# mks0601/ExAvatar_RELEASE

Measured on AMD Instinct MI355X. Metric: train iters/sec (fwd+bwd raster) at 1024x1024 / ~150k Gaussians, higher is better.
Workload: dtype f32

## Files before the change

### exavatar_release_amd/csrc/common.h

```cpp
#pragma once
#include <hip/hip_runtime.h>
#include <stdint.h>
#include "../../include/exa_raster.h"
#include "abi_status.h"

namespace exa {

constexpr int TILE = EXA_RASTER_TILE;
constexpr int SUB = 8;
constexpr int CELL_SUBS = 8;
constexpr int CELL = SUB * CELL_SUBS;
constexpr int SUBS_PER_CELL = CELL_SUBS * CELL_SUBS;
constexpr int BLOCK = 256;
constexpr int CHUNK = 1024;
constexpr int MAX_CELLS = 4096;
constexpr int HEADER_BYTES = 2560;

#ifndef EXA_MAX_BATCH
#define EXA_MAX_BATCH 8
#endif
constexpr int MAX_BATCH = EXA_MAX_BATCH;
template <typename T> struct Batch { T v[MAX_BATCH]; };
template <typename T>
inline Batch<T> make_batch(const T* a, int K) {
    Batch<T> b;
    for (int k = 0; k < MAX_BATCH; ++k) b.v[k] = a[k < K ? k : 0];
    return b;
}

#define EXA_TG_1(a) "s"(a)
#define EXA_TG_2(a, ...) "s"(a), EXA_TG_1(__VA_ARGS__)
#define EXA_TG_3(a, ...) "s"(a), EXA_TG_2(__VA_ARGS__)
#define EXA_TG_4(a, ...) "s"(a), EXA_TG_3(__VA_ARGS__)
#define EXA_TG_5(a, ...) "s"(a), EXA_TG_4(__VA_ARGS__)
#define EXA_TG_6(a, ...) "s"(a), EXA_TG_5(__VA_ARGS__)
#define EXA_TG_7(a, ...) "s"(a), EXA_TG_6(__VA_ARGS__)
#define EXA_TG_8(a, ...) "s"(a), EXA_TG_7(__VA_ARGS__)
#define EXA_TG_9(a, ...) "s"(a), EXA_TG_8(__VA_ARGS__)
#define EXA_TG_10(a, ...) "s"(a), EXA_TG_9(__VA_ARGS__)
#define EXA_TG_11(a, ...) "s"(a), EXA_TG_10(__VA_ARGS__)
#define EXA_TG_12(a, ...) "s"(a), EXA_TG_11(__VA_ARGS__)
#define EXA_TG_13(a, ...) "s"(a), EXA_TG_12(__VA_ARGS__)
#define EXA_TG_14(a, ...) "s"(a), EXA_TG_13(__VA_ARGS__)
#define EXA_TG_15(a, ...) "s"(a), EXA_TG_14(__VA_ARGS__)
#define EXA_TG_16(a, ...) "s"(a), EXA_TG_15(__VA_ARGS__)
#define EXA_TG_17(a, ...) "s"(a), EXA_TG_16(__VA_ARGS__)
#define EXA_TG_18(a, ...) "s"(a), EXA_TG_17(__VA_ARGS__)
#define EXA_TG_19(a, ...) "s"(a), EXA_TG_18(__VA_ARGS__)
#define EXA_TG_20(a, ...) "s"(a), EXA_TG_19(__VA_ARGS__)
#define EXA_TG_21(a, ...) "s"(a), EXA_TG_20(__VA_ARGS__)
#define EXA_TG_22(a, ...) "s"(a), EXA_TG_21(__VA_ARGS__)
#define EXA_TG_23(a, ...) "s"(a), EXA_TG_22(__VA_ARGS__)
#define EXA_TG_24(a, ...) "s"(a), EXA_TG_23(__VA_ARGS__)
#define EXA_TG_TOO_MANY(...) "s"(EXA_TOGETHER_takes_at_most_24_values_behind_the_guard)
#define EXA_TG_PICK(_1, _2, _3, _4, _5, _6, _7, _8, _9, _10, _11, _12, _13, _14, _15, _16, _17, _18, _19, _20, _21, _22, _23, _24, \
                    _25, _26, _27, _28, _29, _30, _31, _32, N, ...) N
#define EXA_TOGETHER(guard, ...)                                                                                            \
    asm("" : "+s"(guard)                                                                                                    \
        : EXA_TG_PICK(__VA_ARGS__, EXA_TG_TOO_MANY, EXA_TG_TOO_MANY, EXA_TG_TOO_MANY, EXA_TG_TOO_MANY, EXA_TG_TOO_MANY,      \
                      EXA_TG_TOO_MANY, EXA_TG_TOO_MANY, EXA_TG_TOO_MANY, EXA_TG_24, EXA_TG_23, EXA_TG_22, EXA_TG_21,         \
                      EXA_TG_20, EXA_TG_19, EXA_TG_18, EXA_TG_17, EXA_TG_16, EXA_TG_15, EXA_TG_14, EXA_TG_13, EXA_TG_12,     \
                      EXA_TG_11, EXA_TG_10, EXA_TG_9, EXA_TG_8, EXA_TG_7, EXA_TG_6, EXA_TG_5, EXA_TG_4, EXA_TG_3, EXA_TG_2,  \
                      EXA_TG_1)(__VA_ARGS__))

__device__ __forceinline__ uint32_t uniform_word(uint32_t v) { return (uint32_t)__builtin_amdgcn_readfirstlane((int)v); }
__device__ __forceinline__ float uniform_word(float v) { return __int_as_float(__builtin_amdgcn_readfirstlane(__float_as_int(v))); }
__device__ __forceinline__ uint4 uniform_word(const uint4& v) {
    return make_uint4(uniform_word(v.x), uniform_word(v.y), uniform_word(v.z), uniform_word(v.w));
}

constexpr float NEAR_CULL = 0.2f;
constexpr float LOWPASS = 0.3f;
constexpr float ALPHA_MAX = 0.99f;
constexpr float ALPHA_MIN = 1.0f / 255.0f;
constexpr float T_EPS = 1e-4f;
constexpr float LOG2E = 1.4426950408889634f;

struct alignas(64) Splat {
    float px, py; uint32_t flags; int32_t radius;
    float ca, cb, cc, opacity;
    float r, g, b, depth;
    uint32_t sub_x, sub_y, n_inst, inst_off;
};
static_assert(sizeof(Splat) == 64, "Splat must be one 64-byte line");

#ifndef EXA_PARTIAL_BYTES
#define EXA_PARTIAL_BYTES 40
#endif
constexpr int PARTIAL_BYTES = EXA_PARTIAL_BYTES;
static_assert(PARTIAL_BYTES == 40 || PARTIAL_BYTES == 48 || PARTIAL_BYTES == 64, "partial records: ten floats packed, three rows, or one 64-byte line");
struct PartialWs { float4* rec; };
typedef float partial_v4 __attribute__((ext_vector_type(4), aligned(8)));
typedef float partial_v2 __attribute__((ext_vector_type(2), aligned(8)));
__device__ __forceinline__ char* partial_at(float4* rec, size_t ps) { return reinterpret_cast<char*>(rec) + ps * PARTIAL_BYTES; }
__device__ __forceinline__ const char* partial_at(const float4* rec, size_t ps) { return reinterpret_cast<const char*>(rec) + ps * PARTIAL_BYTES; }
__device__ __forceinline__ void partial_load(const float4* rec, size_t ps, float4& q0, float4& q1, float4& q2) {
    const char* p = partial_at(rec, ps);
    const partial_v4 a = *reinterpret_cast<const partial_v4*>(p), b = *reinterpret_cast<const partial_v4*>(p + 16);
    q0 = make_float4(a.x, a.y, a.z, a.w); q1 = make_float4(b.x, b.y, b.z, b.w);
    if (PARTIAL_BYTES == 40) {
        const partial_v2 c = *reinterpret_cast<const partial_v2*>(p + 32);
        q2 = make_float4(c.x, c.y, 0.f, 0.f);
    } else {
        const partial_v4 c = *reinterpret_cast<const partial_v4*>(p + 32);
        q2 = make_float4(c.x, c.y, c.z, c.w);
    }
}

struct Grid {
    int W, H;
    int gx, gy;
    int sx, sy;
    int cx, cy, cells;
    int subtiles;
};
__host__ __device__ inline Grid make_grid(int W, int H) {
    Grid g;
    g.W = W; g.H = H;
    g.gx = (W + TILE - 1) / TILE;
    g.gy = (H + TILE - 1) / TILE;
    g.sx = (W + SUB - 1) / SUB;
    g.sy = (H + SUB - 1) / SUB;
    g.cx = (W + CELL - 1) / CELL;
    g.cy = (H + CELL - 1) / CELL;
    g.cells = g.cx * g.cy;
    g.subtiles = g.cells * SUBS_PER_CELL;
    return g;
}

__host__ __device__ inline int num_chunks(int P) { return (P + CHUNK - 1) / CHUNK; }

#ifndef EXA_BIN_PARTS
#define EXA_BIN_PARTS 4
#endif
constexpr int BIN_PARTS = EXA_BIN_PARTS;
struct TileWs {
    ExaRasterHeader* header;
    uint32_t* cls_cur;
    uint32_t* bwd_meta;
    unsigned long long* chunk_cell;
    unsigned long long* cell_cnt;
    uint2* cell_off;
    uint32_t* chunk_inst;
    uint32_t* chunk_vis;
    uint32_t* chunk_tiles;
    uint32_t* chunk_off;
    uint4* cell_desc;
    uint2* ranges;
    uint4* slots;
    uint2* fwd_exit;
    uint32_t* cell_long;
    uint32_t* part_cnt;
    uint4* part_desc;
    uint8_t* cls_code;
};
__host__ __device__ inline uint64_t tile_ws_bytes(int cells, int chunks) {
    return HEADER_BYTES + align256(uint64_t(chunks) * cells * 8) + align256(uint64_t(cells) * 8) +
           align256(uint64_t(cells + 1) * 8) + 4 * align256(uint64_t(chunks + 1) * 4) +
           align256(uint64_t(cells) * 16) + align256(uint64_t(cells) * SUBS_PER_CELL * 8) +
           align256(uint64_t(cells) * SUBS_PER_CELL * 16) + align256(uint64_t(cells) * SUBS_PER_CELL * 8) +
           align256(uint64_t(cells) * BIN_PARTS * SUBS_PER_CELL * 4) + align256(uint64_t(cells) * 4) +
           align256(uint64_t(cells) * BIN_PARTS * 16) + align256(uint64_t(cells) * SUBS_PER_CELL);
}
__host__ __device__ inline TileWs carve_tile_ws(void* base, int cells, int chunks) {
    char* p = static_cast<char*>(base);
    TileWs w;
    w.header = reinterpret_cast<ExaRasterHeader*>(p);
    w.cls_cur = reinterpret_cast<uint32_t*>(p + 256);
    w.bwd_meta = reinterpret_cast<uint32_t*>(p + 128);
    p += HEADER_BYTES;
    w.chunk_cell = reinterpret_cast<unsigned long long*>(p); p += align256(uint64_t(chunks) * cells * 8);
    w.cell_cnt = reinterpret_cast<unsigned long long*>(p); p += align256(uint64_t(cells) * 8);
    w.cell_off = reinterpret_cast<uint2*>(p); p += align256(uint64_t(cells + 1) * 8);
    w.chunk_inst = reinterpret_cast<uint32_t*>(p); p += align256(uint64_t(chunks + 1) * 4);
    w.chunk_vis = reinterpret_cast<uint32_t*>(p); p += align256(uint64_t(chunks + 1) * 4);
    w.chunk_tiles = reinterpret_cast<uint32_t*>(p); p += align256(uint64_t(chunks + 1) * 4);
    w.chunk_off = reinterpret_cast<uint32_t*>(p); p += align256(uint64_t(chunks + 1) * 4);
    w.cell_desc = reinterpret_cast<uint4*>(p); p += align256(uint64_t(cells) * 16);
    w.ranges = reinterpret_cast<uint2*>(p); p += align256(uint64_t(cells) * SUBS_PER_CELL * 8);
    w.slots = reinterpret_cast<uint4*>(p); p += align256(uint64_t(cells) * SUBS_PER_CELL * 16);
    w.fwd_exit = reinterpret_cast<uint2*>(p); p += align256(uint64_t(cells) * SUBS_PER_CELL * 8);
    w.part_cnt = reinterpret_cast<uint32_t*>(p); p += align256(uint64_t(cells) * BIN_PARTS * SUBS_PER_CELL * 4);
    w.cell_long = reinterpret_cast<uint32_t*>(p); p += align256(uint64_t(cells) * 4);
    w.part_desc = reinterpret_cast<uint4*>(p); p += align256(uint64_t(cells) * BIN_PARTS * 16);
    w.cls_code = reinterpret_cast<uint8_t*>(p);
    return w;
}

constexpr int BATCH = 64;
__host__ __device__ inline uint64_t bin_zero_bytes(uint64_t cap) {
    return align256((cap / BATCH + 1) * 16) + align256((cap / BATCH + 1) * 8) + align256(cap);
}
__host__ __device__ inline uint64_t bin_ws_bytes(uint64_t cap) {
    return align256(cap * 8) + align256(cap * 4) + align256(cap * 16) + bin_zero_bytes(cap) +
           align256((cap / BATCH + 1) * 5 * 64 * 4);
}
struct BinWs {
    unsigned long long* keys; uint32_t* sorted; uint4* bucket;
    uint4* owner; unsigned long long* bmask; uint8_t* touched;
    float* ckpt;
};
__host__ __device__ inline BinWs carve_bin_ws(void* base, uint64_t cap) {
    BinWs b;
    char* p = static_cast<char*>(base);
    b.keys = reinterpret_cast<unsigned long long*>(p); p += align256(cap * 8);
    b.sorted = reinterpret_cast<uint32_t*>(p); p += align256(cap * 4);
    b.bucket = reinterpret_cast<uint4*>(p); p += align256(cap * 16);
    b.owner = reinterpret_cast<uint4*>(p); p += align256((cap / BATCH + 1) * 16);
    b.bmask = reinterpret_cast<unsigned long long*>(p); p += align256((cap / BATCH + 1) * 8);
    b.touched = reinterpret_cast<uint8_t*>(p); p += align256(cap);
    b.ckpt = reinterpret_cast<float*>(p);
    return b;
}
__host__ __device__ inline uint32_t cell_slots(uint32_t inst) {
    return inst ? (inst + BATCH - 1) / BATCH + 2 * SUBS_PER_CELL : 0u;
}

__host__ __device__ inline uint64_t grad_ws_bytes(uint64_t cap) { return align256(cap * PARTIAL_BYTES); }
constexpr int GROUP_SCRATCH_FLOATS = 23;
__host__ __device__ inline uint64_t group_scratch_bytes(uint64_t P) { return align256(P * GROUP_SCRATCH_FLOATS * sizeof(float)); }
__host__ __device__ inline PartialWs carve_grad_ws(void* base, uint64_t) {
    PartialWs w;
    w.rec = reinterpret_cast<float4*>(base);
    return w;
}

constexpr int ORDER_CLASSES = 64;
#ifndef EXA_XCD_REGIONS
#define EXA_XCD_REGIONS 8
#endif
constexpr int XCD_REGIONS = EXA_XCD_REGIONS;
static_assert(XCD_REGIONS == 8 || XCD_REGIONS == 1, "eight XCDs, or no regions at all");
__device__ __forceinline__ int xcd_region(int local) { return XCD_REGIONS == 8 ? ((local >> 1) & 3) | ((local >> 3) & 4) : 0; }
constexpr uint32_t BWD_ORDER_MAGIC = 0xB07DE7EDu;
constexpr int BWD_ORDER_DEPTH = 16;
__device__ __forceinline__ int length_class(uint32_t n) { return n ? min(ORDER_CLASSES - 1, (int)((n + 15) / 16)) : 0; }

struct SubTile { int st, cell, local, ox, oy, gsx, gsy; };
__device__ __forceinline__ SubTile decode_subtile(int st, const Grid& g) {
    SubTile s;
    s.st = st;
    s.cell = st >> 6;
    s.local = st & 63;
    const int cxi = s.cell % g.cx, cyi = s.cell / g.cx;
    s.gsx = cxi * CELL_SUBS + (s.local & 7);
    s.gsy = cyi * CELL_SUBS + (s.local >> 3);
    s.ox = s.gsx * SUB;
    s.oy = s.gsy * SUB;
    return s;
}

__device__ __forceinline__ float gauss_power2(float A, float B, float C, float dx, float dy) {
#pragma clang fp contract(off)
    return __builtin_fmaf(A * dx, dx, __builtin_fmaf(C * dy, dy, (B * dx) * dy));
}
__device__ __forceinline__ float gauss_falloff2(float power2) { return __builtin_amdgcn_exp2f(power2); }

struct Footprint { float kA, ysr, X2, D4; bool test; };
__device__ __forceinline__ float clampf(float v, float lo, float hi) { return __builtin_amdgcn_fmed3f(v, lo, hi); }
__device__ __forceinline__ Footprint make_footprint(float A, float B, float C, float opacity, float xm, float ym) {
    Footprint f;
    const float rA = __builtin_amdgcn_rcpf(A), rC = __builtin_amdgcn_rcpf(C);
    const float As = A - 0.25f * B * B * rC;
    f.test = A < 0.f && C < 0.f && As < 0.f;
    const float mag = fabsf(A) * xm * xm + fabsf(B) * xm * ym + fabsf(C) * ym * ym;
    const float thr = -__log2f(255.0f * opacity) - 1e-3f - 1e-5f * mag;
    f.kA = -0.5f * B * rA;
    f.ysr = -0.5f * B * rC * __builtin_amdgcn_sqrtf(thr * __builtin_amdgcn_rcpf(As));
    f.X2 = thr * rA;
    f.D4 = C * As * rA * rA;
    return f;
}
__device__ __forceinline__ bool footprint_band(const Footprint& f, float yl, float yh, float& xa, float& xb) {
    const float yR = clampf(f.ysr, yl, yh), yL = clampf(-f.ysr, yl, yh);
    const float hR2 = f.X2 - f.D4 * yR * yR, hL2 = f.X2 - f.D4 * yL * yL;
    if (hR2 < 0.f || hL2 < 0.f) return false;
    xb = f.kA * yR + __builtin_amdgcn_sqrtf(hR2);
    xa = f.kA * yL - __builtin_amdgcn_sqrtf(hL2);
    return true;
}
__device__ __forceinline__ void wave_lds_fence() {
    asm volatile("s_waitcnt lgkmcnt(0)" ::: "memory");
    __builtin_amdgcn_wave_barrier();
}
struct PreprocessArgs {
    int P, sh_M, sh_degree;
    Grid grid;
    float tanfovx, tanfovy, focal_x, focal_y, scale_modifier;
// ... 135 lines not shown
```

### exavatar_release_amd/csrc/render_fwd.hip

```cpp
#include <stdlib.h>
#include "blend.h"

namespace exa {

constexpr int RBLOCK = 64;

constexpr int SORT_TILE = 2048;
constexpr int SBLOCK = 256;

template <int E>
__device__ __forceinline__ void lds_merge_sort(const unsigned long long* gkeys, int n, uint32_t* __restrict__ sorted,
                                               unsigned long long* keys_out, unsigned long long* buf, int tid) {
    constexpr int NPAD = SBLOCK * E;
    const int lane = tid & 63;
    unsigned long long key[E];
#pragma unroll
    for (int e = 0; e < E; ++e) {
        const int i = e * SBLOCK + tid;
        key[e] = i < n ? gkeys[i] : ~0ull;
        buf[i] = key[e];
    }
    __syncthreads();
    {
        uint32_t rank[E];
// ... 11 lines not shown
        }
        __syncthreads();
#pragma unroll
        for (int e = 0; e < E; ++e) {
            const int i = e * SBLOCK + tid;
            const uint32_t r = (i >= n) ? (uint32_t)lane : rank[e];
            buf[(i & ~63) + r] = key[e];
        }
    }
    __syncthreads();
#pragma unroll
    for (int L = 64, steps = 7; L < NPAD; L <<= 1, ++steps) {
        uint32_t lohi[E];
#pragma unroll
        for (int e = 0; e < E; ++e) {
            key[e] = buf[e * SBLOCK + tid];
            lohi[e] = (uint32_t)L << 16;
        }
        for (int it = 0; it < steps; ++it) {
#pragma unroll
            for (int e = 0; e < E; ++e) {
                const int i = e * SBLOCK + tid;
                const int base = i & ~(2 * L - 1);
                const bool first = (i - base) < L;
                const int p0 = base + (first ? L : 0);
                const int lo = lohi[e] & 0xffff, hi = lohi[e] >> 16;
                const int mid = (lo + hi) >> 1;
                const bool act = lo < hi;
                const unsigned long long pk = buf[p0 + min(mid, L - 1)];
                const bool less = first ? (pk < key[e]) : (pk <= key[e]);
                const int nlo = (act && less) ? mid + 1 : lo;
                const int nhi = (act && !less) ? mid : hi;
                lohi[e] = (uint32_t)nlo | ((uint32_t)nhi << 16);
            }
        }
        __syncthreads();
#pragma unroll
        for (int e = 0; e < E; ++e) {
            const int i = e * SBLOCK + tid;
            const int base = i & ~(2 * L - 1);
            const int off = i - base;
            buf[base + (off < L ? off : off - L) + (int)(lohi[e] & 0xffff)] = key[e];
        }
        __syncthreads();
    }
#pragma unroll
    for (int e = 0; e < E; ++e) {
        const int i = e * SBLOCK + tid;
        if (i < n) {
            sorted[i] = (uint32_t)buf[i];
            if (keys_out) keys_out[i] = buf[i];
        }
    }
}

constexpr int BUCKET_MAX = 48;
template <int E>
__device__ __forceinline__ bool lds_bucket_sort(const unsigned long long* gkeys, int n, uint32_t* __restrict__ sorted,
                                                unsigned long long* keys_out, unsigned long long* buf, uint32_t* cnt,
                                                uint32_t* s_misc, int tid) {
    constexpr int NB = SBLOCK * E;
    const int lane = tid & 63, wave = tid >> 6;
    unsigned long long key[E];
    uint32_t dmin = 0xffffffffu, dmax = 0u;
#pragma unroll
    for (int e = 0; e < E; ++e) key[e] = gkeys[min(e * SBLOCK + tid, n - 1)];
#pragma unroll
    for (int e = 0; e < E; ++e) {
        const int i = e * SBLOCK + tid;
        if (i < n) {
            const uint32_t d = (uint32_t)(key[e] >> 32);
            dmin = min(dmin, d); dmax = max(dmax, d);
        } else {
            key[e] = ~0ull;
        }
        cnt[i] = 0u;
    }
#pragma unroll
    for (int d = 32; d > 0; d >>= 1) {
        dmin = min(dmin, (uint32_t)__shfl_xor((int)dmin, d, 64));
        dmax = max(dmax, (uint32_t)__shfl_xor((int)dmax, d, 64));
    }
    if (lane == 0) { s_misc[wave] = dmin; s_misc[4 + wave] = dmax; }
    __syncthreads();
    dmin = min(min(s_misc[0], s_misc[1]), min(s_misc[2], s_misc[3]));
    dmax = max(max(s_misc[4], s_misc[5]), max(s_misc[6], s_misc[7]));
    const float fmin = __uint_as_float(dmin);
    const float scale = (float)(NB - 1) / fmaxf(__uint_as_float(dmax) - fmin, 1e-30f);
    uint32_t bkt[E], slot[E];
#pragma unroll
    for (int e = 0; e < E; ++e) {
        bkt[e] = 0u; slot[e] = 0u;
        if (e * SBLOCK + tid < n) {
            const float f = (__uint_as_float((uint32_t)(key[e] >> 32)) - fmin) * scale;
            bkt[e] = (uint32_t)min(NB - 1, (int)f);
            slot[e] = __hip_atomic_fetch_add(&cnt[bkt[e]], 1u, __ATOMIC_RELAXED, __HIP_MEMORY_SCOPE_WORKGROUP);
        }
    }
    __syncthreads();
    uint32_t c[E], sum = 0u, mx = 0u;
#pragma unroll
    for (int e = 0; e < E; ++e) { c[e] = cnt[tid * E + e]; sum += c[e]; mx = max(mx, c[e]); }
    uint32_t incl = sum;
#pragma unroll
    for (int d = 1; d < 64; d <<= 1) {
        const uint32_t o = (uint32_t)__shfl_up((int)incl, d, 64);
        if (lane >= d) incl += o;
    }
#pragma unroll
    for (int d = 32; d > 0; d >>= 1) mx = max(mx, (uint32_t)__shfl_xor((int)mx, d, 64));
    if (lane == 63) s_misc[8 + wave] = incl;
    if (lane == 0) s_misc[12 + wave] = mx;
    __syncthreads();
    mx = max(max(s_misc[12], s_misc[13]), max(s_misc[14], s_misc[15]));
    if (mx > (uint32_t)BUCKET_MAX) return false;
    uint32_t run = incl - sum;
    for (int w2 = 0; w2 < wave; ++w2) run += s_misc[8 + w2];
#pragma unroll
    for (int e = 0; e < E; ++e) { cnt[tid * E + e] = run; run += c[e]; }
    __syncthreads();
#pragma unroll
    for (int e = 0; e < E; ++e)
        if (e * SBLOCK + tid < n) buf[cnt[bkt[e]] + slot[e]] = key[e];
    __syncthreads();
#pragma unroll
    for (int e = 0; e < E; ++e) {
        if (e * SBLOCK + tid < n) {
            const uint32_t s0 = cnt[bkt[e]], s1 = bkt[e] + 1u < (uint32_t)NB ? cnt[bkt[e] + 1u] : (uint32_t)n;
            uint32_t rank = s0;
            for (uint32_t j = s0; j < s1; ++j) rank += buf[j] < key[e] ? 1u : 0u;
            sorted[rank] = (uint32_t)key[e];
            if (keys_out) keys_out[rank] = key[e];
        }
    }
    return true;
}

__device__ __forceinline__ void wave_rank_sort64(const unsigned long long* gkeys, int n, uint32_t* __restrict__ sorted,
                                                 unsigned long long* keys_out, unsigned long long* buf, int lane) {
    const unsigned long long mine = lane < n ? gkeys[lane] : ~0ull;
    buf[lane] = mine;
    wave_lds_fence();
    const ulonglong2* s2 = reinterpret_cast<const ulonglong2*>(buf);
    uint32_t rank = 0;
#pragma unroll 8
    for (int j = 0; j < 32; ++j) {
        const ulonglong2 kk = s2[j];
        rank += (kk.x < mine) ? 1u : 0u;
        rank += (kk.y < mine) ? 1u : 0u;
    }
    if (lane < n) {
        sorted[rank] = (uint32_t)mine;
        if (keys_out) keys_out[rank] = mine;
    }
}

template <int R>
__device__ __forceinline__ void rank_sort_list(const unsigned long long* __restrict__ gkeys, int n, int first,
                                               uint32_t* __restrict__ sorted, unsigned long long* s_keys, int tid) {
    unsigned long long mine[R];
    uint32_t rank[R];
#pragma unroll
    for (int r = 0; r < R; ++r) {
        const int i = first + r * SBLOCK + tid;
        mine[r] = i < n ? gkeys[i] : ~0ull;
        rank[r] = 0;
    }
    for (int tile = 0; tile < n; tile += SORT_TILE) {
        const int tn = min(SORT_TILE, n - tile);
        __syncthreads();
        for (int i = tid; i < ((tn + 1) & ~1); i += SBLOCK) s_keys[i] = i < tn ? gkeys[tile + i] : ~0ull;
        __syncthreads();
        const ulonglong2* s2 = reinterpret_cast<const ulonglong2*>(s_keys);
#pragma unroll 4
        for (int j = 0; j < (tn + 1) / 2; ++j) {
            const ulonglong2 kk = s2[j];
#pragma unroll
            for (int r = 0; r < R; ++r) {
                rank[r] += (kk.x < mine[r]) ? 1u : 0u;
                rank[r] += (kk.y < mine[r]) ? 1u : 0u;
            }
        }
    }
#pragma unroll
    for (int r = 0; r < R; ++r)
        if (first + r * SBLOCK + tid < n) sorted[rank[r]] = (uint32_t)mine[r];
}

constexpr int ORDER_WGS = 32;
constexpr int ORDER_BINS = XCD_REGIONS * ORDER_CLASSES;
constexpr int ORDER_LDS_WORDS = 3 * ORDER_BINS + XCD_REGIONS * (BWD_ORDER_DEPTH + 1);
template <typename RangeOf>
__device__ __forceinline__ void order_slots(const TileWs& w, uint32_t* __restrict__ bwd_order, int subtiles, int part, int tid,
                                            uint32_t* __restrict__ lds, RangeOf range_of) {
    uint32_t* const s_off = lds;
    uint32_t* const s_cnt = lds + ORDER_BINS;
    uint32_t* const s_base = lds + 2 * ORDER_BINS;
    uint32_t* const s_bbase = lds + 3 * ORDER_BINS;
    const int lane = tid & 63;
#ifdef EXA_PROBE_SORTLINE
#define ORDER_STAMP(ph) do { if (tid == 0) w.part_cnt[2 * (subtiles + ORDER_WGS) + part * 8 + (ph)] = (uint32_t)wall_clock64(); } while (0)
#else
#define ORDER_STAMP(ph) do {} while (0)
#endif
    ORDER_STAMP(0);
    for (int i = tid; i < ORDER_BINS; i += SBLOCK) s_cnt[i] = 0u;
    __syncthreads();
    const uint4* __restrict__ codes = reinterpret_cast<const uint4*>(w.cls_code);
    const int n16 = subtiles / 16;
    for (int base = 0; base < n16; base += SBLOCK * 4) {
        uint4 v[4];
#pragma unroll
        for (int i = 0; i < 4; ++i) {
            const int idx = base + i * SBLOCK + tid;
            v[i] = idx < n16 ? codes[idx] : make_uint4(0u, 0u, 0u, 0u);
        }
#pragma unroll
        for (int i = 0; i < 4; ++i) {
            const int idx = base + i * SBLOCK + tid;
            const uint32_t word[4] = {v[i].x, v[i].y, v[i].z, v[i].w};
            if ((word[0] | word[1] | word[2] | word[3]) == 0u) continue;
#pragma unroll
            for (int j = 0; j < 16; ++j) {
                const uint32_t cls = (word[j >> 2] >> (8 * (j & 3))) & 0xffu;
                if (cls) atomicAdd(&s_cnt[xcd_region((idx & 3) * 16 + j) * ORDER_CLASSES + cls], 1u);
            }
        }
    }
    __syncthreads();
    ORDER_STAMP(1);
    {
        constexpr int RPW = (XCD_REGIONS + SBLOCK / 64 - 1) / (SBLOCK / 64);
        const int cls = lane == 63 ? 0 : 63 - lane;
        uint32_t v[RPW], incl[RPW];
#pragma unroll
        for (int j = 0; j < RPW; ++j) {
            const int x = (tid >> 6) + j * (SBLOCK / 64);
            v[j] = incl[j] = x < XCD_REGIONS ? s_cnt[x * ORDER_CLASSES + cls] : 0u;
        }
#pragma unroll
        for (int d = 1; d < 64; d <<= 1) {
#pragma unroll
            for (int j = 0; j < RPW; ++j) {
                const uint32_t o = __shfl_up(incl[j], d, 64);
                if (lane >= d) incl[j] += o;
            }
        }
#pragma unroll
        for (int j = 0; j < RPW; ++j) {
            const int x = (tid >> 6) + j * (SBLOCK / 64);
            if (x < XCD_REGIONS) s_off[x * ORDER_CLASSES + cls] = incl[j] - v[j];
        }
    }
    __syncthreads();
    for (int i = tid; i < ORDER_BINS; i += SBLOCK) s_cnt[i] = 0u;
    if (tid < XCD_REGIONS) {
        uint32_t more[BWD_ORDER_DEPTH];
#pragma unroll
        for (int b = 0; b < BWD_ORDER_DEPTH; ++b) more[b] = s_off[tid * ORDER_CLASSES + 4 * b];
        uint32_t run = 0u;
#pragma unroll
        for (int b = 0; b < BWD_ORDER_DEPTH; ++b) { s_bbase[tid * (BWD_ORDER_DEPTH + 1) + b] = run; run += more[b]; }
        s_bbase[tid * (BWD_ORDER_DEPTH + 1) + BWD_ORDER_DEPTH] = run;
    }
    __syncthreads();
    uint32_t M[XCD_REGIONS];
#pragma unroll
    for (int x = 0; x < XCD_REGIONS; ++x) M[x] = s_bbase[x * (BWD_ORDER_DEPTH + 1) + BWD_ORDER_DEPTH];
    uint32_t m_min = M[0], deep_base = M[0];
#pragma unroll
    for (int x = 1; x < XCD_REGIONS; ++x) { m_min = min(m_min, M[x]); deep_base += M[x]; }
    if (part == 0 && tid == 0) { w.bwd_meta[0] = deep_base; w.bwd_meta[2] = bwd_order ? BWD_ORDER_MAGIC : 0u; }
    ORDER_STAMP(2);
    const int per = (subtiles + ORDER_WGS - 1) / ORDER_WGS;
    const int lo = part * per, hi = min(subtiles, lo + per);
    for (int base = lo; base < hi; base += SBLOCK * 4) {
        uint2 r[4];
        uint32_t rank[4];
#pragma unroll
        for (int i = 0; i < 4; ++i) {
            const int st = base + i * SBLOCK + tid;
            r[i] = st < hi ? range_of(st) : make_uint2(0u, 0u);
        }
#pragma unroll
        for (int i = 0; i < 4; ++i) {
            const int st = base + i * SBLOCK + tid;
            const bool valid = st < hi;
            const int cls = length_class(r[i].y - r[i].x), x = xcd_region(st & 63);
            const bool is_empty = valid && cls == 0;
            unsigned long long mine = 0ull;
#pragma unroll
            for (int xr = 0; xr < XCD_REGIONS; ++xr) {
                const unsigned long long m = __ballot(is_empty && x == xr);
                if (x == xr) mine = m;
            }
            const int leader = is_empty ? __ffsll((long long)mine) - 1 : lane;
            uint32_t b0 = 0u;
            if (cls) b0 = atomicAdd(&s_cnt[x * ORDER_CLASSES + cls], 1u);
            else if (is_empty && lane == leader) b0 = atomicAdd(&s_cnt[x * ORDER_CLASSES], (uint32_t)__popcll(mine));
            b0 = (uint32_t)__shfl((int)b0, leader, 64);
            rank[i] = b0 + (is_empty ? (uint32_t)__popcll(mine & ((1ull << lane) - 1ull)) : 0u);
        }
        ORDER_STAMP(3);
        __syncthreads();
        {
            constexpr int BPT = (ORDER_BINS + SBLOCK - 1) / SBLOCK;
            uint32_t c[BPT], got[BPT];
#pragma unroll
            for (int j = 0; j < BPT; ++j) c[j] = j * SBLOCK + tid < ORDER_BINS ? s_cnt[j * SBLOCK + tid] : 0u;
#pragma unroll
            for (int j = 0; j < BPT; ++j) got[j] = c[j] ? atomicAdd(&w.cls_cur[j * SBLOCK + tid], c[j]) : 0u;
#pragma unroll
            for (int j = 0; j < BPT; ++j)
                if (j * SBLOCK + tid < ORDER_BINS) s_base[j * SBLOCK + tid] = s_off[j * SBLOCK + tid] + got[j];
        }
        __syncthreads();
        ORDER_STAMP(4);
#pragma unroll
        for (int i = 0; i < 4; ++i) {
            const int st = base + i * SBLOCK + tid;
            if (st < hi) {
                const int cls = length_class(r[i].y - r[i].x), x = xcd_region(st & 63);
                const uint32_t k = s_base[x * ORDER_CLASSES + cls] + rank[i];
                w.slots[k * XCD_REGIONS + x] = make_uint4(r[i].x, r[i].y, (uint32_t)st, 0u);
                const uint32_t nb = (r[i].y - r[i].x + BATCH - 1) / BATCH, slot0 = r[i].x / BATCH;
                for (uint32_t b = 0; bwd_order && b < nb; ++b) {
                    uint32_t q;
                    if (b < (uint32_t)BWD_ORDER_DEPTH) {
                        const uint32_t kb = s_bbase[x * (BWD_ORDER_DEPTH + 1) + b] + k;
                        q = kb * XCD_REGIONS + (uint32_t)x;
                        if (kb >= m_min) {
                            q = 0u;
#pragma unroll
                            for (int xo = 0; xo < XCD_REGIONS; ++xo) q += min(M[xo], kb) + (xo < x && M[xo] > kb ? 1u : 0u);
                        }
                    } else {
                        q = deep_base + atomicAdd(&w.bwd_meta[1], 1u);
                    }
                    bwd_order[q] = slot0 + b;
                }
            }
        }
        __syncthreads();
        for (int i = tid; i < ORDER_BINS; i += SBLOCK) s_cnt[i] = 0u;
        __syncthreads();
        ORDER_STAMP(5);
    }
#undef ORDER_STAMP
}

__global__ __launch_bounds__(SBLOCK) void sort_short_kernel(Batch<RenderFwdArgs> batch) {
    __shared__ __attribute__((aligned(16))) unsigned long long s_buf[(SBLOCK / 64) * 64];
    const RenderFwdArgs& a = batch.v[blockIdx.y];
    const int wave = threadIdx.x >> 6, lane = threadIdx.x & 63;
    const int idx = (int)blockIdx.x * (SBLOCK / 64) + wave;
    if (idx >= a.grid.subtiles) return;
    if (idx >= (int)a.tw.header->active_cells * SUBS_PER_CELL) return;
    const int st = (int)a.tw.cell_desc[idx >> 6].x * SUBS_PER_CELL + (idx & 63);
    const uint2 range = a.tw.ranges[st];
    const int n = (int)(range.y - range.x);
    if (n > 0 && n <= 64)
        wave_rank_sort64(a.bw.keys + range.x, n, a.bw.sorted + range.x, a.keep_sorted_keys ? a.bw.keys + range.x : nullptr,
                         s_buf + wave * 64, lane);
}

template <bool SPLIT, bool KEEP>
__global__ __launch_bounds__(SBLOCK) __attribute__((amdgpu_waves_per_eu(6, 6))) void sort_subtiles_kernel(Batch<RenderFwdArgs> batch) {
    __shared__ __attribute__((aligned(16))) unsigned long long s_buf[SORT_TILE];
    __shared__ uint32_t s_cnt[SORT_TILE];
    __shared__ uint32_t s_misc[16];
    const RenderFwdArgs& a = batch.v[blockIdx.y];
    if ((int)blockIdx.x >= a.grid.subtiles + ORDER_WGS) return;
    const int tid = threadIdx.x;
#ifdef EXA_PROBE_SORTLINE
    struct TL { const RenderFwdArgs& a; unsigned long long t0; int tid;
        __device__ ~TL() { __syncthreads(); if (tid == 0) { a.tw.part_cnt[2 * blockIdx.x] = (uint32_t)t0; a.tw.part_cnt[2 * blockIdx.x + 1] = (uint32_t)wall_clock64(); } } } tl{a, (unsigned long long)wall_clock64(), tid};
#endif
    if (blockIdx.x < ORDER_WGS) {
        static_assert(ORDER_LDS_WORDS <= SORT_TILE, "order_slots borrows the bucket counters of the sort");
        order_slots(a.tw, a.store_ctx ? reinterpret_cast<uint32_t*>(a.bw.bucket) : nullptr, a.grid.subtiles, (int)blockIdx.x, tid,
                    s_cnt, [&](int st) { return a.tw.ranges[st]; });
        return;
    }
#ifdef EXA_PROBE_SORT
    const unsigned long long t0 = __builtin_readcyclecounter();
#endif
    if (blockIdx.x == ORDER_WGS && tid == 0 && (uint64_t)a.tw.header->num_rendered > a.capacity) a.tw.header->overflow = 1u;
    const int wg = (int)blockIdx.x - ORDER_WGS;
    if (wg >= (int)a.tw.header->active_cells * SUBS_PER_CELL) return;
    if (SPLIT && a.tw.cell_long[wg >> 6] == 0u) return;
    const int st = (int)a.tw.cell_desc[wg >> 6].x * SUBS_PER_CELL + (wg & 63);
    const uint2 range = a.tw.ranges[st];
    const int n = (int)(range.y - range.x);
    if (n == 0) return;
    unsigned long long* gkeys = a.bw.keys + range.x;
    uint32_t* sorted = a.bw.sorted + range.x;
    unsigned long long* const keys_out = KEEP ? gkeys : nullptr;
    if (n <= 64) {
        if (!SPLIT && tid < 64) wave_rank_sort64(gkeys, n, sorted, keys_out, s_buf, tid);
        return;
    }
    if (n > SORT_TILE) {
        for (int first = 0; first < n; first += 8 * SBLOCK) rank_sort_list<8>(gkeys, n, first, sorted, s_buf, tid);
        if (keys_out) {
            __threadfence_block();
            __syncthreads();
            for (int i = tid; i < n; i += SBLOCK) {
                const uint32_t id = sorted[i];
                keys_out[i] = ((unsigned long long)__float_as_uint(a.splats[id].depth) << 32) | id;
            }
        }
        return;
    }
    bool done;
    if (n <= 256) done = lds_bucket_sort<1>(gkeys, n, sorted, keys_out, s_buf, s_cnt, s_misc, tid);
    else if (n <= 512) done = lds_bucket_sort<2>(gkeys, n, sorted, keys_out, s_buf, s_cnt, s_misc, tid);
    else if (n <= 1024) done = lds_bucket_sort<4>(gkeys, n, sorted, keys_out, s_buf, s_cnt, s_misc, tid);
    else done = lds_bucket_sort<8>(gkeys, n, sorted, keys_out, s_buf, s_cnt, s_misc, tid);
    if (done) return;
    __syncthreads();
    if (n <= 256) lds_merge_sort<1>(gkeys, n, sorted, keys_out, s_buf, tid);
    else if (n <= 512) lds_merge_sort<2>(gkeys, n, sorted, keys_out, s_buf, tid);
    else if (n <= 1024) lds_merge_sort<4>(gkeys, n, sorted, keys_out, s_buf, tid);
    else lds_merge_sort<8>(gkeys, n, sorted, keys_out, s_buf, tid);
#ifdef EXA_PROBE_SORT
    __syncthreads();
    if (tid == 0) a.tw.part_cnt[st] = (uint32_t)(__builtin_readcyclecounter() - t0);
#endif
}

template <bool STORE, bool TWO>
__global__ __launch_bounds__(RBLOCK) void render_fwd_kernel(Batch<RenderFwdArgs> batch) {
    __shared__ BatchLds s_b;

    const RenderFwdArgs& a = batch.v[blockIdx.y];
    int subtiles = a.grid.subtiles;
    const int gW = a.grid.W, gH = a.grid.H, gcx = a.grid.cx;
    const uint4* __restrict__ slots = a.tw.slots;
    const Splat* __restrict__ splats = a.splats;
    const uint32_t* __restrict__ sorted_all = a.bw.sorted;
    float* ckpt_all = a.bw.ckpt;
    unsigned long long* bmask = a.bw.bmask;
    uint2* fwd_exit = a.tw.fwd_exit;
    const float* __restrict__ bg = a.bg;
    float* out_color = a.out_color; float* out_depth = a.out_depth; float* out_alpha = a.out_alpha;
    const uint2* ranges = a.tw.ranges;
    const Splat* __restrict__ splats2 = a.splats2;
    const float* src_color = a.src_color; const float* src_depth = a.src_depth; const float* src_alpha = a.src_alpha;
    const float* src_bg = a.src_bg;
    if (TWO)
        EXA_TOGETHER(subtiles, gW, gH, gcx, slots, splats, sorted_all, ckpt_all, bmask, fwd_exit, bg, out_color, out_depth, out_alpha,
                     ranges, splats2, src_color, src_depth, src_alpha, src_bg);
    else
        EXA_TOGETHER(subtiles, gW, gH, gcx, slots, splats, sorted_all, ckpt_all, bmask, fwd_exit, bg, out_color, out_depth, out_alpha);
    if ((int)blockIdx.x >= subtiles) return;
    const int lane = threadIdx.x;
#ifdef EXA_PROBE_FWD
    const unsigned long long t0 = wall_clock64();
#endif
    uint4 slot = uniform_word(slots[blockIdx.x]);
    const float bg0 = uniform_word(bg[0]), bg1 = uniform_word(bg[1]), bg2 = uniform_word(bg[2]);
    EXA_TOGETHER(slot.z, slot.x, slot.y, slot.w, bg0, bg1, bg2);
    Grid grid;
    grid.W = gW; grid.H = gH; grid.cx = gcx;
    const SubTile sub = decode_subtile((int)slot.z, grid);
    const int st = sub.st;
    if (sub.ox >= gW || sub.oy >= gH) return;
    const int pxi = sub.ox + (lane & 7), pyi = sub.oy + (lane >> 3);
    const bool inside = pxi < gW && pyi < gH;
    const float fx = (float)pxi, fy = (float)pyi;
    const uint2 range = TWO ? ranges[slot.z] : make_uint2(slot.x, slot.y);
    const int n = (int)(range.y - range.x);
    if (TWO && n == 0 && reuse_a_pixels(src_color, src_bg, bg0, bg1, bg2)) {
        if (inside) {
            const size_t HW = (size_t)gW * gH, pix = (size_t)pyi * gW + pxi;
            const float c0 = src_color[pix], c1 = src_color[HW + pix], c2 = src_color[2 * HW + pix];
            const float d = src_depth[pix], al = src_alpha[pix];
            out_color[pix] = c0; out_color[HW + pix] = c1; out_color[2 * HW + pix] = c2;
            out_depth[pix] = d; out_alpha[pix] = al;
        }
        if (STORE && lane == 0) fwd_exit[st] = make_uint2(0u, 0u);
        return;
    }

    float T = inside ? 1.0f : 0.0f, Tdead = 1.0f;
    v2f Crg = {0.f, 0.f}, Cbd = {0.f, 0.f};
    const uint32_t* __restrict__ sorted = sorted_all + range.x;
    auto record = [&](uint32_t id) -> const float4* {
        if (TWO) return reinterpret_cast<const float4*>(((id & SRC_B) ? splats2 : splats) + (id & ~SRC_B));
        return reinterpret_cast<const float4*>(splats + id);
    };

    uint32_t id_next = 0;
    float2 r0 = make_float2(0.f, 0.f);
    float4 r1 = make_float4(0.f, 0.f, 0.f, 0.f), r2 = r1;
    if (n > 0) {
        const uint32_t id0 = lane < n ? sorted[lane] : 0u;
        if (64 + lane < n) id_next = sorted[64 + lane];
        if (lane < n) {
            const float4* rec = record(id0);
            r0 = *reinterpret_cast<const float2*>(rec); r1 = rec[1]; r2 = rec[2];
        }
    }
    float* ckpt = ckpt_all + (size_t)(range.x / BATCH) * (5 * 64) + lane;
    int entered = 0;
    for (int base = 0; base < n; base += 64) {
        if (__all(T == 0.0f)) break;
        if (STORE && base > 0) {
            float* c = ckpt + (size_t)entered * (5 * 64);
            c[0] = T > 0.0f ? T : -Tdead; c[64] = Crg.x; c[128] = Crg.y; c[192] = Cbd.x; c[256] = Cbd.y;
        }
        ++entered;
        const unsigned long long unsafe = __builtin_amdgcn_ballot_w64(!conic_safe(r1.x, r1.y, r1.z));
        stage_splat(s_b, lane, r0, r1, r2);
        {
            const int jn = base + 64 + lane;
            r0 = make_float2(0.f, 0.f); r1 = make_float4(0.f, 0.f, 0.f, 0.f); r2 = r1;
            if (jn < n) {
                const float4* rec = record(id_next);
                r0 = *reinterpret_cast<const float2*>(rec); r1 = rec[1]; r2 = rec[2];
            }
            if (jn + 64 < n) id_next = sorted[jn + 64];
        }
        wave_lds_fence();
        const int cnt = min(64, n - base);
        unsigned long long blended = 0ull;
        auto blend4 = [&](const Alpha4& e, const float4& c0, const float4& c1, const float4& c2, const float4& c3, int k) -> bool {
#ifdef EXA_FWD_SKIP_VOTE
            const float amax = fmaxf(fmaxf(e.alpha[0], e.alpha[1]), fmaxf(e.alpha[2], e.alpha[3])) * T;
            if (!__any(amax > 0.0f)) return false;
#endif
            const unsigned long long live_mask = __builtin_amdgcn_ballot_w64(T > 0.0f);
            if (STORE) {
                auto vote_bit = [&](int j, uint32_t bit) -> uint32_t {
                    const unsigned long long m = e.took[j] & live_mask;
                    uint32_t r;
                    asm("s_cmp_lg_u64 %1, 0\n\ts_cselect_b32 %0, %2, 0" : "=s"(r) : "s"(m), "s"(bit) : "scc");
                    return r;
                };
                const uint32_t nib = vote_bit(0, 1u) | vote_bit(1, 2u) | vote_bit(2, 4u) | vote_bit(3, 8u);
                blended |= (unsigned long long)nib << k;
            }
            float Tb[4], w[4];
            blend_group4(T, Tdead, live_mask, e.alpha, Tb, w);
            Crg = __builtin_elementwise_fma(v2f{c0.x, c0.y}, v2f{w[0], w[0]}, Crg);
            Cbd = __builtin_elementwise_fma(v2f{c0.z, c0.w}, v2f{w[0], w[0]}, Cbd);
            Crg = __builtin_elementwise_fma(v2f{c1.x, c1.y}, v2f{w[1], w[1]}, Crg);
            Cbd = __builtin_elementwise_fma(v2f{c1.z, c1.w}, v2f{w[1], w[1]}, Cbd);
            Crg = __builtin_elementwise_fma(v2f{c2.x, c2.y}, v2f{w[2], w[2]}, Crg);
            Cbd = __builtin_elementwise_fma(v2f{c2.z, c2.w}, v2f{w[2], w[2]}, Cbd);
            Crg = __builtin_elementwise_fma(v2f{c3.x, c3.y}, v2f{w[3], w[3]}, Crg);
            Cbd = __builtin_elementwise_fma(v2f{c3.z, c3.w}, v2f{w[3], w[3]}, Cbd);
#ifdef EXA_FWD_EXIT4
            return __all(T == 0.0f);
#else
            return (k & 4) ? __all(T == 0.0f) : false;
#endif
        };
        auto group4 = [&](const Ops4& ops, int k) -> bool {
            const float4 c0 = s_b.col[k], c1 = s_b.col[k + 1], c2 = s_b.col[k + 2], c3 = s_b.col[k + 3];
            Alpha4 e = splat_alpha4(ops, fx, fy, true);
            if ((unsafe >> k) & 0xfull) power_guard4(e, ops, (uint32_t)((unsafe >> k) & 0xfull));
            return blend4(e, c0, c1, c2, c3, k);
        };
        Ops4 opsA = load_ops4(s_b, 0);
        for (int k = 0; k < cnt; k += 8) {
            const Ops4 opsB = load_ops4(s_b, (k + 4) & 63);
            if (group4(opsA, k)) break;
            if (k + 4 >= cnt) break;
            opsA = load_ops4(s_b, (k + 8) & 63);
            if (group4(opsB, k + 4)) break;
        }
        if (STORE && lane == 0) bmask[range.x / BATCH + (uint32_t)(entered - 1)] = blended;
        wave_lds_fence();
    }

    const size_t HW = (size_t)gW * gH;
    if (inside) {
        const size_t pix = (size_t)pyi * gW + pxi;
        const float Tf = T > 0.0f ? T : Tdead;
        out_color[pix] = Crg.x + Tf * bg0;
        out_color[HW + pix] = Crg.y + Tf * bg1;
        out_color[2 * HW + pix] = Cbd.x + Tf * bg2;
        out_depth[pix] = Cbd.y;
        out_alpha[pix] = 1.0f - Tf;
    }
    if (STORE) {
        if (lane == 0) fwd_exit[st] = make_uint2((uint32_t)n, (uint32_t)entered);
#ifdef EXA_PROBE_FWD
        if (lane == 0) {
            a.tw.part_cnt[4 * blockIdx.x] = (uint32_t)t0;
            a.tw.part_cnt[4 * blockIdx.x + 1] = (uint32_t)wall_clock64();
            const uint32_t hw = __builtin_amdgcn_s_getreg((31 << 11) | 4), xcc = __builtin_amdgcn_s_getreg((31 << 11) | 20);
            a.tw.part_cnt[4 * blockIdx.x + 2] = (hw & 0xffffu) | ((xcc & 0xfu) << 16);
        }
#endif
        if (n > 0) {
            float* c = ckpt + (size_t)((n + BATCH - 1) / BATCH) * (5 * 64);
            c[0] = T > 0.0f ? T : Tdead; c[64] = Crg.x; c[128] = Crg.y; c[192] = Cbd.x; c[256] = Cbd.y;
        }
    }
}

static int max_subtiles(const RenderFwdArgs* a, int K) {
    int n = 0;
    for (int k = 0; k < K; ++k) n = max(n, a[k].grid.subtiles);
    return n;
}

hipError_t launch_sort_subtiles(const RenderFwdArgs* a, int K, hipStream_t s) {
    const int subtiles = max_subtiles(a, K);
    if (subtiles == 0) return hipSuccess;
    const int split_at = dev_knobs().split_subtiles;
    bool keep = false;
    for (int k = 0; k < K; ++k) keep = keep || a[k].keep_sorted_keys != 0;
    const dim3 grid(subtiles + ORDER_WGS, K);
    if (subtiles >= split_at) {
        sort_short_kernel<<<dim3((subtiles + SBLOCK / 64 - 1) / (SBLOCK / 64), K), SBLOCK, 0, s>>>(make_batch(a, K));
        if (keep) sort_subtiles_kernel<true, true><<<grid, SBLOCK, 0, s>>>(make_batch(a, K));
        else sort_subtiles_kernel<true, false><<<grid, SBLOCK, 0, s>>>(make_batch(a, K));
    } else {
        if (keep) sort_subtiles_kernel<false, true><<<grid, SBLOCK, 0, s>>>(make_batch(a, K));
        else sort_subtiles_kernel<false, false><<<grid, SBLOCK, 0, s>>>(make_batch(a, K));
    }
    return hipGetLastError();
}

#ifndef EXA_FWD_LDS_PAD
#define EXA_FWD_LDS_PAD 0
#endif
hipError_t launch_render_fwd(const RenderFwdArgs* a, int K, hipStream_t s) {
    const int subtiles = max_subtiles(a, K);
    if (subtiles == 0) return hipSuccess;
    constexpr int pad = EXA_FWD_LDS_PAD;
    if (a[0].splats2) {
        if (a[0].store_ctx) render_fwd_kernel<true, true><<<dim3(subtiles, K), RBLOCK, (size_t)pad, s>>>(make_batch(a, K));
        else render_fwd_kernel<false, true><<<dim3(subtiles, K), RBLOCK, (size_t)pad, s>>>(make_batch(a, K));
    } else if (a[0].store_ctx)
        render_fwd_kernel<true, false><<<dim3(subtiles, K), RBLOCK, (size_t)pad, s>>>(make_batch(a, K));
    else
        render_fwd_kernel<false, false><<<dim3(subtiles, K), RBLOCK, (size_t)pad, s>>>(make_batch(a, K));
    return hipGetLastError();
}

}
```

Measured before the change: 7950.

## Sort small subtile lists per wave and long lists via owner-indexed tail workgroups

Adds a quads sort kernel that is used on the non-split path by default. It packs four subtiles per workgroup, one per wave, and sorts lists of up to 512 keys inside a single wave with a new wave-level bucket sort that falls back to a rank sort. Longer lists are handed to extra tail workgroups that find their lists through the owner slot table. The goal is to stop spending a whole 256-thread workgroup with barriers on each small subtile list. In exchange the grid is sized from capacity, so many tail blocks may exit early, and per-wave LDS regions add pressure.

```diff
diff --git a/exavatar_release_amd/csrc/common.h b/exavatar_release_amd/csrc/common.h
--- a/exavatar_release_amd/csrc/common.h
+++ b/exavatar_release_amd/csrc/common.h
@@ -134,6 +134,11 @@
 #define EXA_BIN_PARTS 4
 #endif
 constexpr int BIN_PARTS = EXA_BIN_PARTS;
+#ifndef EXA_WAVE_KEYS
+#define EXA_WAVE_KEYS 512
+#endif
+constexpr int WAVE_KEYS = EXA_WAVE_KEYS;
+static_assert(WAVE_KEYS == 0 || WAVE_KEYS == 256 || WAVE_KEYS == 512, "EXA_WAVE_KEYS: 0, 256 or 512");
 struct TileWs {
     ExaRasterHeader* header;
     uint32_t* cls_cur;
diff --git a/exavatar_release_amd/csrc/render_fwd.hip b/exavatar_release_amd/csrc/render_fwd.hip
--- a/exavatar_release_amd/csrc/render_fwd.hip
+++ b/exavatar_release_amd/csrc/render_fwd.hip
@@ -187,6 +187,108 @@
     if (lane < n) {
         sorted[rank] = (uint32_t)mine;
         if (keys_out) keys_out[rank] = mine;
+    }
+}
+
+template <int E>
+__device__ __forceinline__ void wave_rank_sort_staged(const unsigned long long (&key)[E], int n, uint32_t* __restrict__ sorted,
+                                                      unsigned long long* keys_out, unsigned long long* buf, int lane) {
+#pragma unroll
+    for (int e = 0; e < E; ++e) buf[e * 64 + lane] = key[e];
+    wave_lds_fence();
+    uint32_t rank[E];
+#pragma unroll
+    for (int e = 0; e < E; ++e) rank[e] = 0u;
+    const ulonglong2* s2 = reinterpret_cast<const ulonglong2*>(buf);
+#pragma unroll 2
+    for (int j = 0; j < (n + 1) / 2; ++j) {
+        const ulonglong2 kk = s2[j];
+#pragma unroll
+        for (int e = 0; e < E; ++e) {
+            rank[e] += (kk.x < key[e]) ? 1u : 0u;
+            rank[e] += (kk.y < key[e]) ? 1u : 0u;
+        }
+    }
+#pragma unroll
+    for (int e = 0; e < E; ++e) {
+        if (e * 64 + lane < n) {
+            sorted[rank[e]] = (uint32_t)key[e];
+            if (keys_out) keys_out[rank[e]] = key[e];
+        }
+    }
+}
+
+template <int E>
+__device__ __forceinline__ void wave_bucket_sort(const unsigned long long* gkeys, int n, uint32_t* __restrict__ sorted,
+                                                 unsigned long long* keys_out, unsigned long long* buf, uint32_t* cnt, int lane) {
+    constexpr int NB = 64 * E;
+    unsigned long long key[E];
+    uint32_t dmin = 0xffffffffu, dmax = 0u;
+#pragma unroll
+    for (int e = 0; e < E; ++e) key[e] = gkeys[min(e * 64 + lane, n - 1)];
+#pragma unroll
+    for (int e = 0; e < E; ++e) {
+        const int i = e * 64 + lane;
+        if (i < n) {
+            const uint32_t d = (uint32_t)(key[e] >> 32);
+            dmin = min(dmin, d); dmax = max(dmax, d);
+        } else {
+            key[e] = ~0ull;
+        }
+        cnt[i] = 0u;
+    }
+#pragma unroll
+    for (int d = 32; d > 0; d >>= 1) {
+        dmin = min(dmin, (uint32_t)__shfl_xor((int)dmin, d, 64));
+        dmax = max(dmax, (uint32_t)__shfl_xor((int)dmax, d, 64));
+    }
+    wave_lds_fence();
+    const float fmin = __uint_as_float(dmin);
+    const float scale = (float)(NB - 1) / fmaxf(__uint_as_float(dmax) - fmin, 1e-30f);
+    uint32_t bs[E];
+#pragma unroll
+    for (int e = 0; e < E; ++e) {
+        bs[e] = 0u;
+        if (e * 64 + lane < n) {
+            const float f = (__uint_as_float((uint32_t)(key[e] >> 32)) - fmin) * scale;
+            const uint32_t bkt = (uint32_t)min(NB - 1, (int)f);
+            bs[e] = bkt | (__hip_atomic_fetch_add(&cnt[bkt], 1u, __ATOMIC_RELAXED, __HIP_MEMORY_SCOPE_WORKGROUP) << 16);
+        }
+    }
+    wave_lds_fence();
+    uint32_t c[E], sum = 0u, mx = 0u;
+#pragma unroll
+    for (int e = 0; e < E; ++e) { c[e] = cnt[lane * E + e]; sum += c[e]; mx = max(mx, c[e]); }
+    uint32_t incl = sum;
+#pragma unroll
+    for (int d = 1; d < 64; d <<= 1) {
+        const uint32_t o = (uint32_t)__shfl_up((int)incl, d, 64);
+        if (lane >= d) incl += o;
+    }
+#pragma unroll
+    for (int d = 32; d > 0; d >>= 1) mx = max(mx, (uint32_t)__shfl_xor((int)mx, d, 64));
+    if (mx > (uint32_t)BUCKET_MAX) {
+        wave_rank_sort_staged<E>(key, n, sorted, keys_out, buf, lane);
+        return;
+    }
+    uint32_t run = incl - sum;
+#pragma unroll
+    for (int e = 0; e < E; ++e) { cnt[lane * E + e] = run; run += c[e]; }
+    wave_lds_fence();
+#pragma unroll
+    for (int e = 0; e < E; ++e)
+        if (e * 64 + lane < n) buf[cnt[bs[e] & 0xffffu] + (bs[e] >> 16)] = key[e];
+    wave_lds_fence();
+#pragma unroll
+    for (int e = 0; e < E; ++e) {
+        if (e * 64 + lane < n) {
+            const uint32_t bkt = bs[e] & 0xffffu;
+            const uint32_t s0 = cnt[bkt], s1 = bkt + 1u < (uint32_t)NB ? cnt[bkt + 1u] : (uint32_t)n;
+            uint32_t rank = s0;
+            for (uint32_t j = s0; j < s1; ++j) rank += buf[j] < key[e] ? 1u : 0u;
+            sorted[rank] = (uint32_t)key[e];
+            if (keys_out) keys_out[rank] = key[e];
+        }
     }
 }
 
@@ -399,6 +501,35 @@
                          s_buf + wave * 64, lane);
 }
 
+template <bool KEEP, int MIN_N>
+__device__ __forceinline__ void sort_list_workgroup(const RenderFwdArgs& a, int n, unsigned long long* gkeys, uint32_t* sorted,
+                                                    unsigned long long* s_buf, uint32_t* s_cnt, uint32_t* s_misc, int tid) {
+    unsigned long long* const keys_out = KEEP ? gkeys : nullptr;
+    if (n > SORT_TILE) {
+        for (int first = 0; first < n; first += 8 * SBLOCK) rank_sort_list<8>(gkeys, n, first, sorted, s_buf, tid);
+        if (keys_out) {
+            __threadfence_block();
+            __syncthreads();
+            for (int i = tid; i < n; i += SBLOCK) {
+                const uint32_t id = sorted[i];
+                keys_out[i] = ((unsigned long long)__float_as_uint(a.splats[id].depth) << 32) | id;
+            }
+        }
+        return;
+    }
+    bool done;
+    if (MIN_N < 256 && n <= 256) done = lds_bucket_sort<1>(gkeys, n, sorted, keys_out, s_buf, s_cnt, s_misc, tid);
+    else if (MIN_N < 512 && n <= 512) done = lds_bucket_sort<2>(gkeys, n, sorted, keys_out, s_buf, s_cnt, s_misc, tid);
+    else if (n <= 1024) done = lds_bucket_sort<4>(gkeys, n, sorted, keys_out, s_buf, s_cnt, s_misc, tid);
+    else done = lds_bucket_sort<8>(gkeys, n, sorted, keys_out, s_buf, s_cnt, s_misc, tid);
+    if (done) return;
+    __syncthreads();
+    if (MIN_N < 256 && n <= 256) lds_merge_sort<1>(gkeys, n, sorted, keys_out, s_buf, tid);
+    else if (MIN_N < 512 && n <= 512) lds_merge_sort<2>(gkeys, n, sorted, keys_out, s_buf, tid);
+    else if (n <= 1024) lds_merge_sort<4>(gkeys, n, sorted, keys_out, s_buf, tid);
+    else lds_merge_sort<8>(gkeys, n, sorted, keys_out, s_buf, tid);
+}
+
 template <bool SPLIT, bool KEEP>
 __global__ __launch_bounds__(SBLOCK) __attribute__((amdgpu_waves_per_eu(6, 6))) void sort_subtiles_kernel(Batch<RenderFwdArgs> batch) {
     __shared__ __attribute__((aligned(16))) unsigned long long s_buf[SORT_TILE];
@@ -435,33 +566,62 @@
         if (!SPLIT && tid < 64) wave_rank_sort64(gkeys, n, sorted, keys_out, s_buf, tid);
         return;
     }
-    if (n > SORT_TILE) {
-        for (int first = 0; first < n; first += 8 * SBLOCK) rank_sort_list<8>(gkeys, n, first, sorted, s_buf, tid);
-        if (keys_out) {
-            __threadfence_block();
-            __syncthreads();
-            for (int i = tid; i < n; i += SBLOCK) {
-                const uint32_t id = sorted[i];
-                keys_out[i] = ((unsigned long long)__float_as_uint(a.splats[id].depth) << 32) | id;
-            }
-        }
+    sort_list_workgroup<KEEP, 64>(a, n, gkeys, sorted, s_buf, s_cnt, s_misc, tid);
+#ifdef EXA_PROBE_SORT
+    __syncthreads();
+    if (tid == 0) a.tw.part_cnt[st] = (uint32_t)(__builtin_readcyclecounter() - t0);
+#endif
+}
+
+template <bool KEEP>
+__global__ __launch_bounds__(SBLOCK) __attribute__((amdgpu_waves_per_eu(6, 6))) void sort_subtiles_quads_kernel(Batch<RenderFwdArgs> batch,
+                                                                                                                int quads) {
+    constexpr int WK = WAVE_KEYS > 0 ? WAVE_KEYS : 256;
+    constexpr int TAIL_STRIDE = WK / BATCH + 1;
+    static_assert(4 * WK * 12 <= SORT_TILE * 12, "four wave regions share the buffers of the workgroup sort");
+    __shared__ __attribute__((aligned(16))) unsigned long long s_buf[SORT_TILE + SORT_TILE / 2];
+    __shared__ uint32_t s_misc[16];
+    uint32_t* const s_cnt = reinterpret_cast<uint32_t*>(s_buf + SORT_TILE);
+    const RenderFwdArgs& a = batch.v[blockIdx.y];
+    const int tid = threadIdx.x;
+#ifdef EXA_PROBE_SORTLINE
+    struct TL { const RenderFwdArgs& a; unsigned long long t0; int tid;
+        __device__ ~TL() { __syncthreads(); if (tid == 0) { a.tw.part_cnt[2 * blockIdx.x] = (uint32_t)t0; a.tw.part_cnt[2 * blockIdx.x + 1] = (uint32_t)wall_clock64(); } } } tl{a, (unsigned long long)wall_clock64(), tid};
+#endif
+    if (blockIdx.x < ORDER_WGS) {
+        static_assert(ORDER_LDS_WORDS <= SORT_TILE, "order_slots borrows the bucket counters of the sort");
+        order_slots(a.tw, a.store_ctx ? reinterpret_cast<uint32_t*>(a.bw.bucket) : nullptr, a.grid.subtiles, (int)blockIdx.x, tid,
+                    s_cnt, [&](int st) { return a.tw.ranges[st]; });
         return;
     }
-    bool done;
-    if (n <= 256) done = lds_bucket_sort<1>(gkeys, n, sorted, keys_out, s_buf, s_cnt, s_misc, tid);
-    else if (n <= 512) done = lds_bucket_sort<2>(gkeys, n, sorted, keys_out, s_buf, s_cnt, s_misc, tid);
-    else if (n <= 1024) done = lds_bucket_sort<4>(gkeys, n, sorted, keys_out, s_buf, s_cnt, s_misc, tid);
-    else done = lds_bucket_sort<8>(gkeys, n, sorted, keys_out, s_buf, s_cnt, s_misc, tid);
-    if (done) return;
-    __syncthreads();
-    if (n <= 256) lds_merge_sort<1>(gkeys, n, sorted, keys_out, s_buf, tid);
-    else if (n <= 512) lds_merge_sort<2>(gkeys, n, sorted, keys_out, s_buf, tid);
-    else if (n <= 1024) lds_merge_sort<4>(gkeys, n, sorted, keys_out, s_buf, tid);
-    else lds_merge_sort<8>(gkeys, n, sorted, keys_out, s_buf, tid);
-#ifdef EXA_PROBE_SORT
-    __syncthreads();
-    if (tid == 0) a.tw.part_cnt[st] = (uint32_t)(__builtin_readcyclecounter() - t0);
-#endif
+    const int q = (int)blockIdx.x - ORDER_WGS;
+    if (q < quads) {
+        if (q == 0 && tid == 0 && (uint64_t)a.tw.header->num_rendered > a.capacity) a.tw.header->overflow = 1u;
+        if (q * 4 >= a.grid.subtiles || q * 4 >= (int)a.tw.header->active_cells * SUBS_PER_CELL) return;
+        const int wave = __builtin_amdgcn_readfirstlane(tid >> 6), lane = tid & 63;
+        const int idx = q * 4 + wave;
+        const int st = (int)a.tw.cell_desc[idx >> 6].x * SUBS_PER_CELL + (idx & 63);
+        const uint2 range = a.tw.ranges[st];
+        const int n = (int)(range.y - range.x);
+        if (n > 0 && n <= WK) {
+            unsigned long long* gkeys = a.bw.keys + range.x;
+            uint32_t* sorted = a.bw.sorted + range.x;
+            unsigned long long* const keys_out = KEEP ? gkeys : nullptr;
+            unsigned long long* const w_buf = s_buf + wave * (WK * 12 / 8);
+            uint32_t* const w_cnt = reinterpret_cast<uint32_t*>(w_buf + WK);
+            if (n <= 64) wave_rank_sort64(gkeys, n, sorted, keys_out, w_buf, lane);
+            else if (n <= 128) wave_bucket_sort<2>(gkeys, n, sorted, keys_out, w_buf, w_cnt, lane);
+            else if (WK == 256 || n <= 256) wave_bucket_sort<4>(gkeys, n, sorted, keys_out, w_buf, w_cnt, lane);
+            else wave_bucket_sort<WK / 64>(gkeys, n, sorted, keys_out, w_buf, w_cnt, lane);
+        }
+        return;
+    }
+    const uint32_t slot = (uint32_t)(q - quads) * (uint32_t)TAIL_STRIDE;
+    if ((uint64_t)slot * BATCH >= a.capacity) return;
+    const uint4 own = a.bw.owner[slot];
+    const int n = (int)own.z;
+    if (own.x == 0u || n <= WK || slot - own.y / BATCH >= (uint32_t)TAIL_STRIDE) return;
+    sort_list_workgroup<KEEP, WK>(a, n, a.bw.keys + own.y, a.bw.sorted + own.y, s_buf, s_cnt, s_misc, tid);
 }
 
 template <bool STORE, bool TWO>
@@ -654,6 +814,14 @@
         sort_short_kernel<<<dim3((subtiles + SBLOCK / 64 - 1) / (SBLOCK / 64), K), SBLOCK, 0, s>>>(make_batch(a, K));
         if (keep) sort_subtiles_kernel<true, true><<<grid, SBLOCK, 0, s>>>(make_batch(a, K));
         else sort_subtiles_kernel<true, false><<<grid, SBLOCK, 0, s>>>(make_batch(a, K));
+    } else if (WAVE_KEYS > 0) {
+        const int quads = (subtiles + SBLOCK / 64 - 1) / (SBLOCK / 64);
+        int tail = 0;
+        for (int k = 0; k < K; ++k)
+            tail = max(tail, (int)((a[k].capacity / BATCH + WAVE_KEYS / BATCH) / (uint64_t)(WAVE_KEYS / BATCH + 1)));
+        const dim3 qgrid(ORDER_WGS + quads + tail, K);
+        if (keep) sort_subtiles_quads_kernel<true><<<qgrid, SBLOCK, 0, s>>>(make_batch(a, K), quads);
+        else sort_subtiles_quads_kernel<false><<<qgrid, SBLOCK, 0, s>>>(make_batch(a, K), quads);
     } else {
         if (keep) sort_subtiles_kernel<false, true><<<grid, SBLOCK, 0, s>>>(make_batch(a, K));
         else sort_subtiles_kernel<false, false><<<grid, SBLOCK, 0, s>>>(make_batch(a, K));
```

Result: faster. 8063, median of 6 (+1.4%).
